# jayin92/Skyfall-GS

Measured on AMD Instinct MI355X. Metric: train-step Gaussians/s (fwd+bwd raster) @1080p, higher is better.
Workload: dtype f32; 1 GPU; configs[1]: synthetic cfg2 scene (SURVEY 8d), N=2000000 Gaussians/GPU, 1920x1080, z ~ U(250, 350), colors_precomp, kernel_size=0.1, subpixel_offset=zeros[H,W,2], dL/dimage and dL/ddepth ~ N(0,1)/P, seed=rank, one scene per GPU; N=2000000, width=1920, height=1080, N_vis=2000000, D_ref_16x16=5856939, D_binned_8x8=6945415, parallelism=scene-per-gpu x1, prewarm_steps=50, settle_steps=0, order=random

## Files before the change

### include/sfgs.h

```cpp
#ifndef SFGS_H
#define SFGS_H

#include <stddef.h>
#include <stdint.h>

#ifdef __cplusplus
extern "C" {
#endif

#define SFGS_ABI_VERSION 23

typedef enum SfgsStatus {
  SFGS_OK = 0,
  SFGS_E_ARG = -1,
  SFGS_E_HIP = -2,
  SFGS_E_CAPACITY = -3,
  SFGS_E_UNSUPPORTED = -4
} SfgsStatus;

#define SFGS_DEPTH_NORMALISED 0
#define SFGS_DEPTH_RAW 1

typedef struct SfgsFrame {
  uint32_t struct_size;
  int32_t image_height;
  int32_t image_width;
  float tanfovx;
  float tanfovy;
  float kernel_size;
  float scale_modifier;
  int32_t sh_degree;
  int32_t sh_coeffs;
  int32_t prefiltered;
// ... 54 lines not shown
  size_t geom_bytes;
  size_t tiles_bytes;
  size_t bins_bytes;
  size_t image_bytes;
  size_t dupgrad_bytes;
  int64_t coarse_bins;
} SfgsRasterSizes;

typedef struct SfgsRasterCounters {
  int64_t num_duplicates;
  int64_t num_duplicates_ref;
  int64_t num_visible;
  int64_t max_tile_list;
  int64_t overflow;
  int64_t max_coarse_bin;
  int64_t num_huge_splats;
  int64_t num_big_chunks;
  int64_t prev_valid;
  int64_t prev_long_tiles;
  int64_t prev_max_tile_list;
  int64_t prev_prefilled;
  int64_t prev_tiles_over_512;
  int64_t max_bin_items;
} SfgsRasterCounters;

int sfgs_abi_version(void);
const char* sfgs_last_error(void);

int sfgs_set_option(const char* key, const char* value);
const char* sfgs_get_option(const char* key);

int sfgs_profile_enable(int32_t on);
int sfgs_profile_select(uint64_t kernel_mask);
int sfgs_profile_kernel_count(void);
const char* sfgs_profile_kernel_name(int32_t id);
int sfgs_profile_collect(double* ms_sum, int64_t* launches, int32_t n);

int sfgs_box_probe(double* valu_tflops, double* sclk_mhz_effective, void* stream);

int sfgs_raster_sizes(int32_t N, int32_t W, int32_t H, int64_t D, int64_t coarse_capacity,
                      SfgsRasterSizes* out);
int64_t sfgs_raster_slot_capacity(int32_t W, int32_t H, int64_t num_duplicates);

int sfgs_raster_forward_plan(const SfgsFrame* frame, const SfgsGaussians* g, int32_t* radii,
                             void* geom, size_t geom_bytes, void* tiles, size_t tiles_bytes,
                             void* bins, size_t bins_bytes, int64_t dup_capacity,
// ... 243 lines not shown
```

### skyfall-gs_amd/csrc/api.cpp

```cpp
#include <hip/hip_runtime.h>
#include <stdarg.h>
#include <stdio.h>

#include <stdlib.h>
#include <string.h>

#include <atomic>
#include <mutex>
#include <vector>

#include "../../include/sfgs.h"
#include "sfgs_internal.h"

namespace sfgs {
static thread_local char g_err[512] = "";
void set_error(const char* fmt, ...) {
  va_list ap;
  va_start(ap, fmt);
  vsnprintf(g_err, sizeof(g_err), fmt, ap);
  va_end(ap);
}

struct OptSpec { const char* key; const char* env; const char* values[6]; };
static const OptSpec kOpts[OPT_COUNT] = {
    {"sort", "SFGS_SORT", {"auto", "fused", "fused1024", "split", "fused768", nullptr}},
    {"plan_scan", "SFGS_PLAN_SCAN", {"fused", "separate", nullptr}},
    {"binning", "SFGS_BINNING", {"auto", "direct", nullptr}},
    {"prefill", "SFGS_PREFILL", {"auto", "always", "never", nullptr}},
    {"knn", "SFGS_KNN", {"auto", "brute", nullptr}},
    {"tile_order", "SFGS_TILE_ORDER", {"auto", "always", "never", nullptr}}};
static std::atomic<int> g_opt[OPT_COUNT];
static int opt_value(int which, const char* v) {
  for (int i = 0; v && kOpts[which].values[i]; ++i)
    if (!strcmp(v, kOpts[which].values[i])) return i;
  return -1;
}
static const bool g_opt_init = [] {
  for (int k = 0; k < OPT_COUNT; ++k) {
    const int v = opt_value(k, getenv(kOpts[k].env));
    g_opt[k].store(v < 0 ? 0 : v, std::memory_order_relaxed);
  }
  return true;
}();
int option(int which) { return g_opt[which].load(std::memory_order_relaxed); }

static const char* const kKernelNames[KID_COUNT] = {
    "subpix_bound", "preprocess", "bin_count", "bin_rank", "bin_scatter", "plan_scan", "fine_bin", "sort_tiles_small", "sort_tiles_reg_long",
    "sort_tiles_lds", "composite_fwd", "composite_bwd", "preprocess_bwd", "ssim_fwd", "ssim_mean", "ssim_bwd",
    "knn_dist2", "prepass_fwd", "prepass_bwd", "filter3d", "densify_stats", "adam", "sh_eval_fwd", "sh_eval_bwd", "compact_scan", "compact_gather", "densify",
    "opacity_entropy_fwd", "opacity_entropy_final", "opacity_entropy_bwd",
    "loss_photo_fwd", "loss_depth_fwd", "loss_final", "loss_photo_bwd", "loss_depth_bwd"};

struct ProfRec { int id; hipEvent_t a, b; };
// ... 92 lines not shown
```

### skyfall-gs_amd/csrc/raster_fwd.hip

```cpp
#include <stdlib.h>
#include <string.h>

#include <algorithm>

#include <type_traits>

#include "act_math.h"
#include "sfgs_internal.h"

namespace sfgs {

constexpr int REG_SORT_SMALL = 512;
constexpr int REG_SORT_MAX = 1024;

__global__ void __launch_bounds__(256) subpix_bound_kernel(const float* __restrict__ subpix, int64_t n,
                                                           unsigned long long* __restrict__ hdr) {
  __shared__ float s_m[4];
  float m = 0.f;
  const int64_t n4 = (reinterpret_cast<uintptr_t>(subpix) & 15) ? 0 : (n >> 2);
  const float4* __restrict__ v4 = reinterpret_cast<const float4*>(subpix);
  for (int64_t i = (int64_t)blockIdx.x * blockDim.x + threadIdx.x; i < n4; i += (int64_t)gridDim.x * blockDim.x) {
    const float4 v = v4[i];
    m = fmaxf(fmaxf(m, fmaxf(fabsf(v.x), fabsf(v.y))), fmaxf(fabsf(v.z), fabsf(v.w)));
  }
// ... 894 lines not shown
}

template <int EPL, int SIZE, int STEP>
__device__ __forceinline__ void bitonic_steps(unsigned long long (&key)[EPL], unsigned (&pay)[EPL], int lane) {
  if constexpr (STEP == 0 || (SIZE >> (STEP + 1)) >= 1) {
    bitonic_stage<EPL, SIZE, STEP>(key, pay, lane);
    bitonic_steps<EPL, SIZE, STEP + 1>(key, pay, lane);
  }
}

template <int EPL, int SIZE>
__device__ __forceinline__ void bitonic_sizes(unsigned long long (&key)[EPL], unsigned (&pay)[EPL], int lane) {
  if constexpr (SIZE <= 64 * EPL) {
    bitonic_steps<EPL, SIZE, 0>(key, pay, lane);
    bitonic_sizes<EPL, SIZE * 2>(key, pay, lane);
  }
}

template <int EPL>
__device__ __forceinline__ void wave_bitonic_sort(unsigned long long (&key)[EPL], unsigned (&pay)[EPL], int lane) {
  bitonic_sizes<EPL, 2>(key, pay, lane);
}

template <int EPL>
__device__ __forceinline__ void store_list_entries(uint32_t* __restrict__ dst, const unsigned (&v)[EPL]) {
  if constexpr (EPL >= 4) {
#pragma unroll
    for (int i = 0; i < EPL / 4; ++i)
      reinterpret_cast<uint4*>(dst)[i] = make_uint4(v[4 * i], v[4 * i + 1], v[4 * i + 2], v[4 * i + 3]);
  } else if constexpr (EPL == 2) {
    *reinterpret_cast<uint2*>(dst) = make_uint2(v[0], v[1]);
  } else {
    dst[0] = v[0];
  }
}

template <int EPL>
__device__ __forceinline__ void sort_tile_in_registers(unsigned s, int L, int lane, const uint4* __restrict__ items,
                                                       uint32_t* __restrict__ sorted_id,
                                                       uint32_t* __restrict__ sorted_dup) {
  unsigned long long key[EPL];
  unsigned pay[EPL];
  uint4 it[EPL];
#pragma unroll
  for (int r = 0; r < EPL; ++r) it[r] = items[s + min(r * 64 + lane, L - 1)];
#pragma unroll
// ... 16 lines not shown
__global__ void __launch_bounds__(256)
sort_tiles_reg_kernel(int T8, const uint2* __restrict__ tile_range, const uint4* __restrict__ items,
                      uint32_t* __restrict__ sorted_id, uint32_t* __restrict__ sorted_dup,
                      const unsigned long long* __restrict__ hdr, unsigned long long* __restrict__ feedback) {
  if (feedback && blockIdx.x == 0 && threadIdx.x == 0) {
    feedback[FB_VALID] = 1ull;
    feedback[FB_LONG_TILES] = hdr[HDR_LONG_COUNT];
    feedback[FB_MAX_LIST] = hdr[HDR_MAX_LIST];
    feedback[FB_OVER_512] = hdr[HDR_LONG_COUNT];
  }
  const int t = blockIdx.x * 4 + (threadIdx.x >> 6), lane = threadIdx.x & 63;
  if (t >= T8) return;
  const uint2 tr = tile_range[t];
  const int L = (int)tr.y;
  if (L == 0 || L > REG_SORT_SMALL) return;
  if (L <= 64) sort_tile_in_registers<1>(tr.x, L, lane, items, sorted_id, sorted_dup);
  else if (L <= 128) sort_tile_in_registers<2>(tr.x, L, lane, items, sorted_id, sorted_dup);
  else if (L <= 256) sort_tile_in_registers<4>(tr.x, L, lane, items, sorted_id, sorted_dup);
  else sort_tile_in_registers<8>(tr.x, L, lane, items, sorted_id, sorted_dup);
}

template <int SS_CAP>
struct alignas(16) SelectSortLds {
  unsigned long long key[SS_CAP];
  uint32_t pay[SS_CAP];
  uint32_t pad_[4];
};


template <int SS_CAP>
__global__ void __launch_bounds__(256)
select_sort_kernel(int TX8, int TY8, int CX, int NCB, uint32_t* __restrict__ coarse_count,
                   const uint4* __restrict__ csr, const uint4* __restrict__ slabs, unsigned coarse_capacity,
                   unsigned long long slot_capacity,
                   uint2* __restrict__ tile_range, uint4* __restrict__ items, uint32_t* __restrict__ long_tiles,
                   unsigned long long* __restrict__ hdr, uint32_t* __restrict__ sorted_id,
                   uint32_t* __restrict__ sorted_dup) {
  __shared__ SelectSortLds<SS_CAP> lds_all[COARSE];
  __shared__ unsigned s_cnt[COARSE];
  const unsigned lb = xcd_chunked(blockIdx.x, (unsigned)NCB * COARSE, 8u * COARSE);
  const int cb = (int)(lb / COARSE), q = (int)(lb % COARSE);
  const int tid = threadIdx.x;
  const int wave = __builtin_amdgcn_readfirstlane(tid >> 6), lane = tid & 63;
  const int tx = (cb % CX) * COARSE + wave, ty = (cb / CX) * COARSE + q;
  if (ty >= TY8) return;
  const int t = ty * TX8 + tx;
  const int bit = q * COARSE + wave;
  uint32_t* line = coarse_count + (size_t)cb * CC_STRIDE;
  const BinItems slab = bin_items(line, csr, slabs, (size_t)cb, coarse_capacity);
  const unsigned n = slab.n;
  if (n == 0) { if (lane == 0 && tx < TX8) tile_range[t] = make_uint2(0u, 0u); return; }
  SelectSortLds<SS_CAP>& lds = lds_all[wave];
  if (tid < COARSE) s_cnt[tid] = 0u;
  __syncthreads();
  constexpr int R = 8;
  const unsigned rowmask = 0xfu << (q * COARSE);
  for (unsigned i0 = 0; i0 < n; i0 += 256u * R) {
    uint4 it[R];
#pragma unroll
    for (int k = 0; k < R; ++k) it[k] = slab[min(i0 + 256u * k + tid, n - 1u)];
#pragma unroll
    for (int k = 0; k < R; ++k) {
      unsigned m = i0 + 256u * k + tid < n ? it[k].w & rowmask : 0u;
      while (m) {
        const int b = __builtin_ctz(m);
        m &= m - 1;
        const unsigned pos = atomicAdd(&s_cnt[b - q * COARSE], 1u);
        if (pos < (unsigned)SS_CAP) {
          SelectSortLds<SS_CAP>& dst = lds_all[b - q * COARSE];
          dst.key[pos] = ((unsigned long long)it[k].y << 32) | it[k].x;
          dst.pay[pos] = it[k].z + (unsigned)__popc(it[k].w & ((1u << b) - 1u));
        }
      }
    }
  }
  __syncthreads();
  if (tx >= TX8) return;
  const unsigned below = (1u << bit) - 1u;
  const unsigned c = __builtin_amdgcn_readfirstlane((int)s_cnt[wave]);
  const unsigned long long bin_base = line[2];
  const unsigned need = bin_slots_needed(line[1]);
  const bool dropped = bin_base + need > slot_capacity;
  unsigned off = 0;
  if (lane == 0) {
    if (dropped) hdr[HDR_OVERFLOW] = 1ull;
    else if (c) {
      off = atomicAdd(&line[3], (c + LIST_ALIGN - 1) & ~(unsigned)(LIST_ALIGN - 1));
      atomicMax(&line[4], c);
      if (c > (unsigned)REG_SORT_SMALL) atomicAdd(&line[5], 1u);
    }
  }
  if (dropped || c == 0) { if (lane == 0) tile_range[t] = make_uint2(0u, 0u); return; }
  if (c <= (unsigned)SS_CAP) {
    const int L = (int)c;
    auto finish = [&](auto epl_tag) {
      constexpr int EPL = decltype(epl_tag)::value;
      unsigned long long key[EPL];
      unsigned pay[EPL];
#pragma unroll
      for (int r = 0; r < EPL; ++r) {
        const int i = r * 64 + lane;
        const unsigned long long k = lds.key[min(i, SS_CAP - 1)];
        const unsigned p = lds.pay[min(i, SS_CAP - 1)];
        key[r] = i < L ? k : ~0ull;
        pay[r] = i < L ? p : 0u;
      }
      wave_bitonic_sort<EPL>(key, pay, lane);
      const unsigned s = (unsigned)bin_base + (unsigned)__builtin_amdgcn_readfirstlane((int)off);
      if (lane == 0) tile_range[t] = make_uint2(s, c);
      if (lane * EPL < ((L + LIST_ALIGN - 1) & ~(LIST_ALIGN - 1))) {
        unsigned ids[EPL];
#pragma unroll
        for (int r = 0; r < EPL; ++r) ids[r] = (unsigned)(key[r] & 0xffffffffull);
        store_list_entries<EPL>(sorted_id + s + lane * EPL, ids);
        store_list_entries<EPL>(sorted_dup + s + lane * EPL, pay);
      }
    };
    if (L <= 64) finish(std::integral_constant<int, 1>{});
    else if (L <= 128) finish(std::integral_constant<int, 2>{});
    else if (L <= 256) finish(std::integral_constant<int, 4>{});
    else if (SS_CAP <= 512 || L <= 512) finish(std::integral_constant<int, 8>{});
    else if constexpr (SS_CAP > 512) finish(std::integral_constant<int, 16>{});
    return;
  }
  const unsigned s = (unsigned)bin_base + (unsigned)__builtin_amdgcn_readfirstlane((int)off);
  if (lane == 0) {
    tile_range[t] = make_uint2(s, c);
    long_tiles[atomicAdd(&hdr[HDR_LONG_COUNT], 1ull)] = (unsigned)t;
  }
  unsigned done = 0;
  for (unsigned i0 = 0; i0 < n; i0 += 64u * R) {
    uint4 lt[R];
#pragma unroll
    for (int k = 0; k < R; ++k) lt[k] = slab[min(i0 + 64u * k + lane, n - 1u)];
#pragma unroll
    for (int k = 0; k < R; ++k) {
      const bool hit = i0 + 64u * k + lane < n && ((lt[k].w >> bit) & 1u);
      const unsigned long long b = __ballot(hit);
      const unsigned pos = done + __builtin_amdgcn_mbcnt_hi((unsigned)(b >> 32), __builtin_amdgcn_mbcnt_lo((unsigned)b, 0u));
      if (hit) items[s + pos] = make_uint4(lt[k].x, lt[k].y, lt[k].z + (unsigned)__popc(lt[k].w & below), 0u);
      done += (unsigned)__popcll(b);
    }
  }
}

__device__ void list_stats(int NCB, uint32_t* __restrict__ coarse_count, unsigned long long* hdr,
                           unsigned long long* __restrict__ feedback) {
  __shared__ unsigned ls_part[4], ls_over[4];
  unsigned m = 0, over = 0;
  for (int i = threadIdx.x; i < NCB; i += 256) {
    m = max(m, coarse_count[(size_t)i * CC_STRIDE + 4]);
    over += coarse_count[(size_t)i * CC_STRIDE + 5];
  }
#pragma unroll
  for (int d = 32; d >= 1; d >>= 1) {
    m = max(m, (unsigned)__shfl_xor((int)m, d));
    over += (unsigned)__shfl_xor((int)over, d);
  }
  if ((threadIdx.x & 63) == 0) { ls_part[threadIdx.x >> 6] = m; ls_over[threadIdx.x >> 6] = over; }
  __syncthreads();
  if (threadIdx.x == 0) {
    const unsigned long long mx = max(max(ls_part[0], ls_part[1]), max(ls_part[2], ls_part[3]));
    hdr[HDR_MAX_LIST] = mx;
    if (feedback) {
      feedback[FB_VALID] = 1ull;
      feedback[FB_LONG_TILES] = hdr[HDR_LONG_COUNT];
      feedback[FB_MAX_LIST] = mx;
      feedback[FB_OVER_512] = (unsigned long long)ls_over[0] + ls_over[1] + ls_over[2] + ls_over[3];
    }
  }
  __syncthreads();
}

template <int EPL>
__global__ void __launch_bounds__(256)
sort_tiles_reg_long_kernel(const uint32_t* __restrict__ long_tiles, const unsigned long long* __restrict__ hdr,
                           const uint2* __restrict__ tile_range, const uint4* __restrict__ items,
                           uint32_t* __restrict__ sorted_id, uint32_t* __restrict__ sorted_dup) {
  const unsigned n_long = (unsigned)hdr[HDR_LONG_COUNT];
  const int wave = __builtin_amdgcn_readfirstlane((int)(threadIdx.x >> 6)), lane = threadIdx.x & 63;
  for (unsigned li = blockIdx.x * 4 + wave; li < n_long; li += gridDim.x * 4) {
    const uint2 tr = tile_range[long_tiles[li]];
    const int L = (int)tr.y;
    if (L > 32 * EPL && L <= 64 * EPL) sort_tile_in_registers<EPL>(tr.x, L, lane, items, sorted_id, sorted_dup);
  }
}
// ... 734 lines not shown
  const BinsView bv = bins_view(bins, dup_capacity, NCB, coarse_capacity);
  SFGS_CHECK_HIP(zero_head(tiles, tv.zero_bytes, stream));
  if (frame->subpixel_offset) {
    const int64_t n = (int64_t)W * H * 2;
    const int blocks = (int)std::max<int64_t>(1, std::min<int64_t>((n / 4 + 255) / 256, 512));
    hipLaunchKernelGGL(subpix_bound_kernel, dim3(blocks), dim3(256), 0, stream, frame->subpixel_offset, n, tv.hdr);
  }
  if (N > 0) hipLaunchKernelGGL(plan_merge_rec_kernel, dim3(2048), dim3(256), 0, stream, mp, gv.rec);
  hipLaunchKernelGGL(plan_merge_items_kernel, dim3((unsigned)NCB), dim3(256), 0, stream, mp, (unsigned)export_capacity,
                     (unsigned)coarse_capacity, tv.coarse_count, bv.slabs, tv.hdr);
  hipLaunchKernelGGL(bin_base_scan_kernel, dim3(1), dim3(1024), 0, stream, (int)NCB, tv.coarse_count, tv.hdr);
  SFGS_POST_LAUNCH("plan_merge", stream, frame->debug);
  return SFGS_OK;
}

static void unpack_counters(const unsigned long long* h, SfgsRasterCounters* out) {
  out->num_duplicates = (int64_t)h[HDR_D_EFF];
  out->num_duplicates_ref = (int64_t)h[HDR_D_REF];
  out->num_visible = (int64_t)h[HDR_N_VIS];
  out->max_tile_list = (int64_t)h[HDR_MAX_LIST];
  out->overflow = (int64_t)h[HDR_OVERFLOW];
  out->max_coarse_bin = (int64_t)h[HDR_MAX_COARSE];
  out->max_bin_items = (int64_t)h[HDR_MAX_BIN_ITEMS];
  out->num_huge_splats = (int64_t)h[HDR_BIG_COUNT];
  out->num_big_chunks = (int64_t)h[HDR_BIG_CHUNKS];
  out->prev_valid = out->prev_long_tiles = out->prev_max_tile_list = out->prev_prefilled = out->prev_tiles_over_512 = 0;
}

extern "C" int sfgs_raster_counters_decode(const void* host_128, SfgsRasterCounters* out) {
  SFGS_REQUIRE(host_128 && out, SFGS_E_ARG, "NULL argument");
  const unsigned long long* h = (const unsigned long long*)host_128;
  unsigned long long hdr[HDR_WORDS] = {0};
  for (int i = 0; i < 8; ++i) hdr[i] = h[i];
  hdr[HDR_BIG_COUNT] = h[8];
  hdr[HDR_BIG_CHUNKS] = h[9];
  unpack_counters(hdr, out);
  out->prev_valid = (int64_t)h[10];
  out->prev_long_tiles = (int64_t)h[11];
  out->prev_max_tile_list = (int64_t)h[12];
  out->prev_prefilled = (int64_t)h[13];
  out->prev_tiles_over_512 = (int64_t)h[14];
  out->max_bin_items = (int64_t)h[15];
  return SFGS_OK;
}

extern "C" int sfgs_raster_read_counters(const void* tiles, SfgsRasterCounters* out, void* stream_) {
// ... 25 lines not shown
                                          int64_t num_duplicates, float* out_color, float* out_depth, float* out_alpha,
                                          void* image, size_t image_sz, void* stream_) {
  if (int rc = check_frame(frame)) return rc;
  hipStream_t stream = (hipStream_t)stream_;
  const int W = frame->image_width, H = frame->image_height;
  const int64_t NCB = coarse_bins(W, H);
  SFGS_REQUIRE(N >= 0 && tiles && out_color && out_depth && out_alpha && bins, SFGS_E_ARG, "NULL argument");
  SFGS_REQUIRE(dup_capacity >= 0 && dup_capacity < (1ll << 32) && coarse_capacity >= 0, SFGS_E_ARG, "bad capacity");
  SFGS_REQUIRE(num_duplicates < 0 || sfgs_raster_slot_capacity(W, H, num_duplicates) <= dup_capacity, SFGS_E_CAPACITY,
               "%lld duplicates need %lld list slots, dup_capacity is %lld: redo the plan with larger blobs",
               (long long)num_duplicates, (long long)sfgs_raster_slot_capacity(W, H, num_duplicates),
               (long long)dup_capacity);
  SFGS_REQUIRE(bins_sz >= bins_bytes(dup_capacity, NCB, coarse_capacity), SFGS_E_CAPACITY,
               "bins blob: %zu bytes given, %zu needed", bins_sz, bins_bytes(dup_capacity, NCB, coarse_capacity));
  SFGS_REQUIRE(image == nullptr || image_sz >= image_bytes(W, H, dup_capacity), SFGS_E_CAPACITY, "image blob too small");
  const TilesView tv = tiles_view(tiles, W, H, N, nullptr);
  const GeomView gv = geom_view(const_cast<void*>(geom), N);
  const BinsView bv = bins_view_csr(bins, dup_capacity, NCB, coarse_capacity, N);
  const KFrame kf = make_kframe(frame);
  const int TX8 = tiles8_x(W), TY8 = tiles8_y(H), T8 = TX8 * TY8, CX = coarse_x(W);
  const int fused_cap = sort_fused(frame->launch_hints);
  const bool fused = fused_cap != 0;
  if (fused) {
    { ProfScope ps_(KID_SORT_SMALL, stream);
      if (fused_cap > 768)
        hipLaunchKernelGGL(select_sort_kernel<1024>, dim3((unsigned)NCB * COARSE), dim3(256), 0, stream, TX8, TY8, CX,
                           (int)NCB, tv.coarse_count, bv.csr, bv.slabs, (unsigned)coarse_capacity,
                           (unsigned long long)dup_capacity, tv.tile_range, bv.items, tv.long_tiles, tv.hdr, bv.sorted_id,
                           bv.sorted_dup);
      else if (fused_cap > 512)
        hipLaunchKernelGGL(select_sort_kernel<768>, dim3((unsigned)NCB * COARSE), dim3(256), 0, stream, TX8, TY8, CX,
                           (int)NCB, tv.coarse_count, bv.csr, bv.slabs, (unsigned)coarse_capacity,
                           (unsigned long long)dup_capacity, tv.tile_range, bv.items, tv.long_tiles, tv.hdr, bv.sorted_id,
                           bv.sorted_dup);
      else
        hipLaunchKernelGGL(select_sort_kernel<512>, dim3((unsigned)NCB * COARSE), dim3(256), 0, stream, TX8, TY8, CX,
                           (int)NCB, tv.coarse_count, bv.csr, bv.slabs, (unsigned)coarse_capacity,
                           (unsigned long long)dup_capacity, tv.tile_range, bv.items, tv.long_tiles, tv.hdr, bv.sorted_id,
                           bv.sorted_dup); }
    SFGS_POST_LAUNCH("select_sort", stream, frame->debug);
  } else {
    { ProfScope ps_(KID_FINE_BIN, stream);
      hipLaunchKernelGGL(fine_bin_kernel, dim3((unsigned)NCB), dim3(256), 0, stream, TX8, TY8, CX, (int)NCB,
                         tv.coarse_count, bv.csr, bv.slabs, (unsigned)coarse_capacity, (unsigned long long)dup_capacity,
                         tv.tile_range, bv.items, tv.long_tiles, tv.hdr); }
    SFGS_POST_LAUNCH("fine_bin", stream, frame->debug);
  }
  if (num_duplicates != 0) {
    if (!fused) {
      { ProfScope ps_(KID_SORT_SMALL, stream);
        hipLaunchKernelGGL(sort_tiles_reg_kernel, dim3((T8 + 3) / 4), dim3(256), 0, stream, T8, tv.tile_range, bv.items,
                           bv.sorted_id, bv.sorted_dup, (const unsigned long long*)tv.hdr,
                           (unsigned long long*)frame->feedback); }
      SFGS_POST_LAUNCH("sort_tiles_small", stream, frame->debug);
    }
    const int stats_bins = fused ? (int)NCB : 0;
    if (frame->launch_hints & SFGS_HINT_FEW_LONG_LISTS) {
      ProfScope ps_(KID_SORT_LDS, stream);
      hipLaunchKernelGGL(sort_tiles_long_kernel<SORT_CAP>, dim3(std::min(T8, 768)), dim3(256), 0, stream, REG_SORT_SMALL,
                         tv.long_tiles, tv.hdr, tv.tile_range, bv.items, bv.sorted_id, bv.sorted_dup, stats_bins,
                         tv.coarse_count, tv.hdr, (unsigned long long*)frame->feedback);
    } else {
// ... 88 lines not shown
```

### skyfall-gs_amd/csrc/raster_math.h

```cpp
#pragma once
#include <math.h>
#include <stdint.h>

#ifdef __HIPCC__
#define SFGS_HD __host__ __device__ __forceinline__
#else
#define SFGS_HD static inline
#endif

namespace sfgs {

constexpr int TILE_REF = 16;
constexpr int TILE_BIN = 8;
constexpr float LOG2E = 1.4426950408889634f;
constexpr float LN2 = 0.6931471805599453f;

struct FrameParams {
  int W, H;
  float tanfovx, tanfovy, kernel_size, scale_modifier;
  int sh_degree, sh_coeffs, depth_mode;
  float view[16], proj[16], campos[3], bg[3];
};

struct SplatRec {
// ... 3 lines not shown
  float depth, r;
  float g, b;
  float ex, ey;
};

struct Projected {
  bool visible;
  int radius;
  int rminx, rminy, rmaxx, rmaxy;
  float mx, my;
  float a, b, c;
  float a0, b0, c0;
  float cA, cB, cC;
  float coef;
  float tx, ty, tz;
  float cov3d[6];
};

SFGS_HD int f2i_sat(float v) {
  if (v >= 2147483520.0f) return 2147483647;
  if (v <= -2147483648.0f) return (-2147483647 - 1);
  return (int)v;
}
SFGS_HD int imin(int a, int b) { return a < b ? a : b; }
SFGS_HD int imax(int a, int b) { return a > b ? a : b; }

SFGS_HD void quat_to_rot(const float* q, float R[9]) {
  const float r = q[0], x = q[1], y = q[2], z = q[3];
  R[0] = 1.f - 2.f * (y * y + z * z);
  R[1] = 2.f * (x * y - r * z);
  R[2] = 2.f * (x * z + r * y);
  R[3] = 2.f * (x * y + r * z);
  R[4] = 1.f - 2.f * (x * x + z * z);
  R[5] = 2.f * (y * z - r * x);
  R[6] = 2.f * (x * z - r * y);
  R[7] = 2.f * (y * z + r * x);
  R[8] = 1.f - 2.f * (x * x + y * y);
}

SFGS_HD void cov3d_of(const float* s, float mod, const float* q, float cov[6]) {
  float R[9];
  quat_to_rot(q, R);
  const float S0 = mod * s[0], S1 = mod * s[1], S2 = mod * s[2];
  const float M0 = R[0] * S0, M1 = R[1] * S1, M2 = R[2] * S2;
  const float M3 = R[3] * S0, M4 = R[4] * S1, M5 = R[5] * S2;
  const float M6 = R[6] * S0, M7 = R[7] * S1, M8 = R[8] * S2;
// ... 625 lines not shown
```

### skyfall-gs_amd/csrc/sfgs_internal.h

```cpp
#pragma once
#include <hip/hip_runtime.h>
#include <stdint.h>
#include <stdio.h>

#include "../../include/sfgs.h"
#include "raster_math.h"

namespace sfgs {

void set_error(const char* fmt, ...);

#define SFGS_CHECK_HIP(expr)                                                              \
  do {                                                                                    \
    hipError_t e_ = (expr);                                                               \
    if (e_ != hipSuccess) {                                                               \
      sfgs::set_error("%s failed: %s (%s:%d)", #expr, hipGetErrorString(e_), __FILE__, __LINE__); \
      return SFGS_E_HIP;                                                                  \
    }                                                                                     \
  } while (0)

#define SFGS_REQUIRE(cond, code, ...)  \
  do {                                 \
    if (!(cond)) {                     \
      sfgs::set_error(__VA_ARGS__);    \
      return (code);                   \
    }                                  \
  } while (0)

enum KernelId {
  KID_SUBPIX = 0, KID_PREPROCESS, KID_BIN_COUNT, KID_BIN_RANK, KID_BIN_SCATTER, KID_PLAN_SCAN, KID_FINE_BIN, KID_SORT_SMALL, KID_SORT_REG_LONG, KID_SORT_LDS,
  KID_COMPOSITE_FWD, KID_COMPOSITE_BWD, KID_PREPROCESS_BWD, KID_SSIM_FWD, KID_SSIM_MEAN, KID_SSIM_BWD, KID_KNN, KID_PREPASS_FWD, KID_PREPASS_BWD, KID_FILTER3D, KID_DENSIFY_STATS, KID_ADAM, KID_SH_EVAL_FWD, KID_SH_EVAL_BWD, KID_COMPACT_SCAN, KID_COMPACT_GATHER, KID_DENSIFY,
  KID_OPACITY_ENTROPY_FWD, KID_OPACITY_ENTROPY_FINAL, KID_OPACITY_ENTROPY_BWD,
  KID_LOSS_PHOTO_FWD, KID_LOSS_DEPTH_FWD, KID_LOSS_FINAL, KID_LOSS_PHOTO_BWD, KID_LOSS_DEPTH_BWD,
  KID_COUNT
};
enum { OPT_SORT, OPT_PLAN_SCAN, OPT_BINNING, OPT_PREFILL, OPT_KNN, OPT_TILE_ORDER, OPT_COUNT };
enum { SORT_AUTO = 0, SORT_FUSED = 1, SORT_FUSED1024 = 2, SORT_SPLIT = 3, SORT_FUSED768 = 4 };
enum { PREFILL_AUTO = 0, PREFILL_ALWAYS = 1, PREFILL_NEVER = 2 };
int option(int which);
bool prof_enabled();
bool prof_selected(int id);
void* prof_begin(int id, hipStream_t stream);
void prof_end(void* token, hipStream_t stream);
struct ProfScope {
  void* tok; hipStream_t st;
  ProfScope(int id, hipStream_t s) : tok(prof_selected(id) ? prof_begin(id, s) : nullptr), st(s) {}
  ~ProfScope() { if (tok) prof_end(tok, st); }
};

#define SFGS_POST_LAUNCH(name, stream, debug)                                      \
  do {                                                                             \
    hipError_t e_ = hipGetLastError();                                             \
    if (e_ == hipSuccess && (debug)) e_ = hipStreamSynchronize(stream);            \
    if (e_ != hipSuccess) {                                                        \
      sfgs::set_error("kernel %s failed: %s", name, hipGetErrorString(e_));        \
      return SFGS_E_HIP;                                                           \
    }                                                                              \
  } while (0)

static inline size_t align_up(size_t v, size_t a) { return (v + a - 1) / a * a; }
// ... 36 lines not shown
  for (int i = 0; i < 3; ++i) { f.campos[i] = k.campos[i]; f.bg[i] = k.bg[i]; }
  return f;
}

constexpr int PRE_BLOCK = 256;
enum { FB_VALID = 0, FB_LONG_TILES = 1, FB_MAX_LIST = 2, FB_PREFILLED = 3, FB_OVER_512 = 4 };
constexpr int HDR_WORDS = 64;

enum HeaderSlot {
  HDR_D_EFF = 0,
  HDR_D_REF = 1,
  HDR_N_VIS = 2,
  HDR_MAX_LIST = 3,
  HDR_OVERFLOW = 4,
  HDR_SUBPIX_BOUND = 5,
  HDR_ITEM_ALLOC = 6,
  HDR_MAX_COARSE = 7,
  HDR_LONG_COUNT = 8,
  HDR_BIG_CHUNKS = 9,
  HDR_BIG_COUNT = 10,
  HDR_PREFILLED = 11,
  HDR_CSR_CURSOR = 12,
  HDR_MAX_BIN_ITEMS = 13,
  HDR_TILE_ORDER = 14
};

constexpr int REC_F4 = 3;

struct GeomView {
  float4* rec;
  uint2* dup;
  uint4* big_list;
  uint32_t* block_items;
};
constexpr int PAIRS_PER_BLOCK = PRE_BLOCK * 6;
static inline size_t pairs_bytes(int64_t N) {
  const int64_t NB = (N + PRE_BLOCK - 1) / PRE_BLOCK;
  return align_up((size_t)NB * PAIRS_PER_BLOCK * 16, 256);
}
static inline size_t geom_bytes(int64_t N) {
  const int64_t NB = (N + PRE_BLOCK - 1) / PRE_BLOCK;
  return align_up((size_t)N * 16 * REC_F4, 256) + align_up((size_t)N * 8, 256) + align_up((size_t)N * 16, 256) +
         align_up((size_t)NB * 4, 256);
}
static inline GeomView geom_view(void* base, int64_t N) {
  GeomView g;
  const int64_t NB = (N + PRE_BLOCK - 1) / PRE_BLOCK;
// ... 338 lines not shown
```

### skyfall-gs_amd/diff_gauss/__init__.py

```python
import os
from typing import NamedTuple, Optional

import torch
import torch.nn as nn

from sfgs import _lib as L
from sfgs import features as _features, max_radii as _max_radii, prepass, sh as _sh, viewdirs as _viewdirs
from sfgs import affinity as _affinity

__all__ = ["GaussianRasterizationSettings", "GaussianRasterizer", "rasterize_gaussians", "last_counters",
           "last_backward_hints", "collect_full_counters"]


class GaussianRasterizationSettings(NamedTuple):
    image_height: int
    image_width: int
    tanfovx: float
    tanfovy: float
    kernel_size: float
    subpixel_offset: Optional[torch.Tensor]
    bg: torch.Tensor
    scale_modifier: float
    viewmatrix: torch.Tensor
    projmatrix: torch.Tensor
# ... 271 lines not shown
                frame.feedback = hs["fb"].data_ptr()
            pin, ev, pin_ptr, ev_handle, cnt = _pinned_counters(dev, stream)
            outs_ptr = outs.data_ptr()
            plane = 4 * H * W
            tries, pool_grown, attempts = 0, False, 0
            while True:
                attempts += 1
                total = _layout(lib, N, W, H, cap, ccap, need_bwd)[0]
                if total > _scratch_budget(dev):
                    raise RuntimeError(f"rasterizer scratch of {total / 2**30:.1f} GiB exceeds half of the device memory "
                                       f"(duplicates {cap}, fullest coarse bin {ccap}, {ncb} bins)")
                scratch = torch.empty(total, dtype=torch.uint8, device=dev)
                frame.launch_hints = fwd_hints
                L.check(lib.sfgs_raster_forward(frame, gs, radii.data_ptr(), scratch.data_ptr(), total, cap, ccap,
                                                int(need_bwd), pin_ptr, ev_handle, outs_ptr, outs_ptr + 3 * plane,
                                                outs_ptr + 4 * plane, stream))
                ev.synchronize()
                L.check(lib.sfgs_raster_counters_decode(pin_ptr, cnt))
                if _stats["full"]:
                    full = L.SfgsRasterCounters()
                    tiles_off = _tiles_offset(lib, N, W, H, cap, ccap, need_bwd)
                    L.check(lib.sfgs_raster_read_counters(scratch.data_ptr() + tiles_off, L.C.byref(full), stream))
                    cnt.max_tile_list = full.max_tile_list
                D, cmax = int(cnt.num_duplicates), int(cnt.max_coarse_bin)
                if (fwd_hints & HINT_NO_HUGE_SPLATS) and cnt.num_huge_splats:
                    fwd_hints &= ~HINT_NO_HUGE_SPLATS
                    continue
                if not cnt.overflow and D + over <= cap and cmax <= ccap:
                    break
                tries += 1
                if tries > 24:
                    raise RuntimeError(f"rasterizer plan still overflows after {tries} attempts (duplicates {D}, capacity "
                                       f"{cap}, fullest coarse bin {cmax} of {ccap})")
                new_cap, new_ccap = max(cap, int(D * 1.25) + 1024 + over), max(ccap, int(cmax * 1.25) + 256)
                if (new_cap, new_ccap) == (cap, ccap):
                    new_cap = cap * 2
                    pool_grown = True
                cap, ccap = new_cap, new_ccap
            if hs is not None:
                if cnt.prev_valid:
                    hs["long"] = int(cnt.prev_long_tiles)
                    hs["maxlist"] = int(cnt.prev_max_tile_list)
                    hs["over512"] = int(cnt.prev_tiles_over_512)
                    if hs["prefill_ran"]:
                        hs["prefilled"] = _next_prefilled(hs["prefilled"], int(cnt.prev_prefilled) != 0)
                hs["huge"] = _next_huge(hs["huge"], int(cnt.num_huge_splats))
                hs["cmax"] = int(cnt.max_bin_items)
                hs["D"] = D
                hs["prefill_ran"] = False
            _cap_hint[(di, W, H)] = _next_capacities(cap, ccap, D, cmax, over, pool_grown)
            global _last_counters
            _last_counters = dict(num_duplicates=D, num_duplicates_ref=int(cnt.num_duplicates_ref),
                                  num_visible=int(cnt.num_visible), max_coarse_bin=cmax, max_bin_items=int(cnt.max_bin_items),
                                  num_huge_splats=int(cnt.num_huge_splats), num_big_chunks=int(cnt.num_big_chunks), plan_attempts=attempts,
                                  max_tile_list=int(cnt.max_tile_list), N=N, W=W, H=H, dup_capacity=cap,
                                  coarse_capacity=ccap, fwd_hints=int(fwd_hints))
        finally:
            if switch:
                torch.cuda.set_device(prev_dev)
        color, depth, alpha = outs.split_with_sizes((3, 1, 1))
        norm = _zero(dev).expand(3, H, W)
        ctx.mark_non_differentiable(radii, norm)
        ctx.set_materialize_grads(False)
        if need_bwd:
            ctx.st = (frame, gs, keep, cap, ccap, D, int(cnt.num_big_chunks), hkey, sh_coeffs, colors_precomp is not None,
                      shs is not None, opacities.dtype, total, settings, bool(sh_channel_major))
            ctx.save_for_backward(means3D, scales, rotations, opacities, colors_precomp, shs, radii, scratch, filter_3D,
                                  sh_dirs, shs_rest, sh_centers)
        return color, depth, norm, alpha, radii

    @staticmethod
    def backward(ctx, g_color, g_depth, g_norm, g_alpha, g_radii):
        lib = L.load()
        (means3D, scales, rotations, opacities, colors_precomp, shs, radii, scratch, filter_3D, sh_dirs,
         shs_rest, sh_centers) = ctx.saved_tensors
        (frame0, gs, keep, cap, ccap, ndup, big_chunks, hkey, K, has_colors, has_shs, opac_dtype, total, settings, sh_cm) = ctx.st
        dev = means3D.device
        di = dev.index
# ... 211 lines not shown
```

### skyfall-gs_amd/sfgs/_lib.py

```python
import ctypes as C
import os

_HERE = os.path.dirname(os.path.abspath(__file__))
LIB_PATH = os.environ.get("SFGS_LIB") or os.path.join(_HERE, "libsfgs.so")
ABI_VERSION = 23

SFGS_OK = 0
DEPTH_NORMALISED, DEPTH_RAW = 0, 1


class SfgsFrame(C.Structure):
    _fields_ = [("struct_size", C.c_uint32), ("image_height", C.c_int32), ("image_width", C.c_int32),
                ("tanfovx", C.c_float), ("tanfovy", C.c_float), ("kernel_size", C.c_float),
                ("scale_modifier", C.c_float), ("sh_degree", C.c_int32), ("sh_coeffs", C.c_int32),
                ("prefiltered", C.c_int32), ("debug", C.c_int32), ("depth_mode", C.c_int32),
                ("tile_row_begin", C.c_int32), ("tile_row_end", C.c_int32),
                ("subpixel_offset", C.c_void_p), ("bg", C.c_void_p), ("viewmatrix", C.c_void_p),
                ("projmatrix", C.c_void_p), ("campos", C.c_void_p), ("launch_hints", C.c_uint32),
                ("feedback", C.c_void_p)]


class SfgsGaussians(C.Structure):
    _fields_ = [("struct_size", C.c_uint32), ("count", C.c_int32), ("means3D", C.c_void_p), ("scales", C.c_void_p),
                ("rotations", C.c_void_p), ("opacities", C.c_void_p), ("colors_precomp", C.c_void_p),
                ("shs", C.c_void_p), ("filter_3D", C.c_void_p), ("raw_f64_mask", C.c_int32),
                ("sh_dirs", C.c_void_p), ("shs_channel_major", C.c_int32),
                ("shs_rest", C.c_void_p),
                ("sh_centers", C.c_void_p)]
# ... 68 lines not shown

class SfgsDsmViewArgs(C.Structure):
    _fields_ = [("struct_size", C.c_uint32), ("H", C.c_int32), ("W", C.c_int32), ("depth", C.c_void_p), ("mask", C.c_void_p),
                ("M", C.c_double * 9), ("c", C.c_double * 3), ("origin", C.c_double * 3), ("cx_pix", C.c_double),
                ("cy_pix", C.c_double), ("focal_x", C.c_double), ("focal_y", C.c_double), ("xoff", C.c_double),
                ("yoff_top", C.c_double), ("resolution", C.c_double), ("xsize", C.c_int32), ("ysize", C.c_int32),
                ("mode", C.c_int32), ("radius", C.c_int32)]


class SfgsDsmrArgs(C.Structure):
    _fields_ = [("struct_size", C.c_uint32), ("ref_h", C.c_int32), ("ref_w", C.c_int32), ("sec_h", C.c_int32),
                ("sec_w", C.c_int32), ("ref", C.c_void_p), ("sec", C.c_void_p), ("irange", C.c_int32), ("scaling", C.c_int32),
                ("init_dx", C.c_int32), ("init_dy", C.c_int32)]


DSM_MAX, DSM_MEAN = 0, 1


class SfgsRasterCounters(C.Structure):
    _fields_ = [("num_duplicates", C.c_int64), ("num_duplicates_ref", C.c_int64), ("num_visible", C.c_int64),
                ("max_tile_list", C.c_int64), ("overflow", C.c_int64), ("max_coarse_bin", C.c_int64),
                ("num_huge_splats", C.c_int64), ("num_big_chunks", C.c_int64), ("prev_valid", C.c_int64),
                ("prev_long_tiles", C.c_int64), ("prev_max_tile_list", C.c_int64), ("prev_prefilled", C.c_int64),
                ("prev_tiles_over_512", C.c_int64), ("max_bin_items", C.c_int64)]


_V, _I32, _I64, _SZ = C.c_void_p, C.c_int32, C.c_int64, C.c_size_t
SYMBOLS = {
    "sfgs_abi_version": (C.c_int, []),
    "sfgs_last_error": (C.c_char_p, []),
    "sfgs_profile_enable": (C.c_int, [_I32]),
    "sfgs_profile_select": (C.c_int, [C.c_uint64]),
    "sfgs_set_option": (C.c_int, [C.c_char_p, C.c_char_p]),
    "sfgs_get_option": (C.c_char_p, [C.c_char_p]),
    "sfgs_profile_kernel_count": (C.c_int, []),
    "sfgs_profile_kernel_name": (C.c_char_p, [_I32]),
    "sfgs_profile_collect": (C.c_int, [C.POINTER(C.c_double), C.POINTER(C.c_int64), _I32]),
    "sfgs_box_probe": (C.c_int, [C.POINTER(C.c_double), C.POINTER(C.c_double), _V]),
    "sfgs_raster_sizes": (C.c_int, [_I32, _I32, _I32, _I64, _I64, C.POINTER(SfgsRasterSizes)]),
    "sfgs_raster_slot_capacity": (C.c_int64, [_I32, _I32, _I64]),
    "sfgs_raster_forward_plan": (C.c_int, [C.POINTER(SfgsFrame), C.POINTER(SfgsGaussians), _V, _V, _SZ, _V, _SZ, _V, _SZ,
                                            _I64, _I64, _V, _V]),
    "sfgs_raster_counters_decode": (C.c_int, [_V, C.POINTER(SfgsRasterCounters)]),
    "sfgs_raster_read_counters": (C.c_int, [_V, C.POINTER(SfgsRasterCounters), _V]),
    "sfgs_raster_read_counters_pinned": (C.c_int, [_V, _V, C.POINTER(SfgsRasterCounters), _V]),
    "sfgs_raster_forward_render": (C.c_int, [C.POINTER(SfgsFrame), _I32, _V, _V, _V, _SZ, _I64, _I64, _I64, _V, _V, _V,
                                              _V, _SZ, _V]),
# ... 129 lines not shown
```

Baseline: 2.180 billion Gaussians/s.

## Sort per-tile lists with packed 32-bit depth-position keys in fused select sort

In the fused select-sort kernel, depth is rebased to the wave's minimum and packed with the list position into a single 32-bit key. Lists of up to 512 entries are then sorted with a 32-bit bitonic sort instead of a 64-bit key plus payload sort, which halves shuffle traffic and register use. The LDS layout is split into a depth array and an id/payload pair that is gathered after the sort. If the depth range does not fit or equal depths tie, the tile falls back to the wide sort, which is counted in a new header counter.

```diff
diff --git a/include/sfgs.h b/include/sfgs.h
--- a/include/sfgs.h
+++ b/include/sfgs.h
@@ -8,7 +8,7 @@
 extern "C" {
 #endif
 
-#define SFGS_ABI_VERSION 23
+#define SFGS_ABI_VERSION 24
 
 typedef enum SfgsStatus {
   SFGS_OK = 0,
@@ -109,6 +109,7 @@
   int64_t prev_prefilled;
   int64_t prev_tiles_over_512;
   int64_t max_bin_items;
+  int64_t sort_wide_tiles;
 } SfgsRasterCounters;
 
 int sfgs_abi_version(void);
diff --git a/skyfall-gs_amd/csrc/api.cpp b/skyfall-gs_amd/csrc/api.cpp
--- a/skyfall-gs_amd/csrc/api.cpp
+++ b/skyfall-gs_amd/csrc/api.cpp
@@ -28,7 +28,8 @@
     {"binning", "SFGS_BINNING", {"auto", "direct", nullptr}},
     {"prefill", "SFGS_PREFILL", {"auto", "always", "never", nullptr}},
     {"knn", "SFGS_KNN", {"auto", "brute", nullptr}},
-    {"tile_order", "SFGS_TILE_ORDER", {"auto", "always", "never", nullptr}}};
+    {"tile_order", "SFGS_TILE_ORDER", {"auto", "always", "never", nullptr}},
+    {"sort_key", "SFGS_SORT_KEY", {"auto", "wide", "narrow", nullptr}}};
 static std::atomic<int> g_opt[OPT_COUNT];
 static int opt_value(int which, const char* v) {
   for (int i = 0; v && kOpts[which].values[i]; ++i)
diff --git a/skyfall-gs_amd/csrc/raster_fwd.hip b/skyfall-gs_amd/csrc/raster_fwd.hip
--- a/skyfall-gs_amd/csrc/raster_fwd.hip
+++ b/skyfall-gs_amd/csrc/raster_fwd.hip
@@ -940,6 +940,64 @@
   bitonic_sizes<EPL, 2>(key, pay, lane);
 }
 
+template <int EPL, int SIZE, int STEP>
+__device__ __forceinline__ void bitonic_stage(unsigned (&key)[EPL], int lane) {
+  constexpr int mask = STEP == 0 ? SIZE - 1 : (SIZE >> (STEP + 1));
+  constexpr int rmask = mask & (EPL - 1);
+  constexpr int lmask = mask / EPL;
+  if constexpr (lmask == 0) {
+#pragma unroll
+    for (int r = 0; r < EPL; ++r) {
+      const int q = r ^ rmask;
+      if (q > r) {
+        const unsigned kr = key[r], kq = key[q];
+        key[r] = min(kr, kq); key[q] = max(kr, kq);
+      }
+    }
+  } else {
+    const bool upper = (lane & (lmask & ~(lmask >> 1))) != 0;
+    unsigned nk[EPL];
+#pragma unroll
+    for (int r = 0; r < EPL; ++r) {
+      const unsigned theirs = xor_shuffle<lmask>(key[r ^ rmask]);
+      nk[r] = upper ? max(key[r], theirs) : min(key[r], theirs);
+    }
+#pragma unroll
+    for (int r = 0; r < EPL; ++r) key[r] = nk[r];
+  }
+}
+
+template <int EPL, int SIZE, int STEP>
+__device__ __forceinline__ void bitonic_steps(unsigned (&key)[EPL], int lane) {
+  if constexpr (STEP == 0 || (SIZE >> (STEP + 1)) >= 1) {
+    bitonic_stage<EPL, SIZE, STEP>(key, lane);
+    bitonic_steps<EPL, SIZE, STEP + 1>(key, lane);
+  }
+}
+
+template <int EPL, int SIZE>
+__device__ __forceinline__ void bitonic_sizes(unsigned (&key)[EPL], int lane) {
+  if constexpr (SIZE <= 64 * EPL) {
+    bitonic_steps<EPL, SIZE, 0>(key, lane);
+    bitonic_sizes<EPL, SIZE * 2>(key, lane);
+  }
+}
+
+template <int EPL>
+__device__ __forceinline__ void wave_bitonic_sort(unsigned (&key)[EPL], int lane) {
+  bitonic_sizes<EPL, 2>(key, lane);
+}
+
+__device__ __forceinline__ unsigned wave_min_u32(unsigned v) {
+  v = min(v, xor_shuffle<1>(v));
+  v = min(v, xor_shuffle<2>(v));
+  v = min(v, xor_shuffle<7>(v));
+  v = min(v, xor_shuffle<15>(v));
+  const unsigned a = (unsigned)__builtin_amdgcn_readlane((int)v, 0), b = (unsigned)__builtin_amdgcn_readlane((int)v, 16);
+  const unsigned c = (unsigned)__builtin_amdgcn_readlane((int)v, 32), d = (unsigned)__builtin_amdgcn_readlane((int)v, 48);
+  return min(min(a, b), min(c, d));
+}
+
 template <int EPL>
 __device__ __forceinline__ void store_list_entries(uint32_t* __restrict__ dst, const unsigned (&v)[EPL]) {
   if constexpr (EPL >= 4) {
@@ -1002,8 +1060,8 @@
 
 template <int SS_CAP>
 struct alignas(16) SelectSortLds {
-  unsigned long long key[SS_CAP];
-  uint32_t pay[SS_CAP];
+  uint2 idp[SS_CAP];
+  uint32_t depth[SS_CAP];
   uint32_t pad_[4];
 };
 
@@ -1015,7 +1073,7 @@
                    unsigned long long slot_capacity,
                    uint2* __restrict__ tile_range, uint4* __restrict__ items, uint32_t* __restrict__ long_tiles,
                    unsigned long long* __restrict__ hdr, uint32_t* __restrict__ sorted_id,
-                   uint32_t* __restrict__ sorted_dup) {
+                   uint32_t* __restrict__ sorted_dup, int narrow) {
   __shared__ SelectSortLds<SS_CAP> lds_all[COARSE];
   __shared__ unsigned s_cnt[COARSE];
   const unsigned lb = xcd_chunked(blockIdx.x, (unsigned)NCB * COARSE, 8u * COARSE);
@@ -1048,8 +1106,8 @@
         const unsigned pos = atomicAdd(&s_cnt[b - q * COARSE], 1u);
         if (pos < (unsigned)SS_CAP) {
           SelectSortLds<SS_CAP>& dst = lds_all[b - q * COARSE];
-          dst.key[pos] = ((unsigned long long)it[k].y << 32) | it[k].x;
-          dst.pay[pos] = it[k].z + (unsigned)__popc(it[k].w & ((1u << b) - 1u));
+          dst.depth[pos] = it[k].y;
+          dst.idp[pos] = make_uint2(it[k].x, it[k].z + (unsigned)__popc(it[k].w & ((1u << b) - 1u)));
         }
       }
     }
@@ -1075,20 +1133,68 @@
     const int L = (int)c;
     auto finish = [&](auto epl_tag) {
       constexpr int EPL = decltype(epl_tag)::value;
+      const bool owns = lane * EPL < ((L + LIST_ALIGN - 1) & ~(LIST_ALIGN - 1));
+      if (narrow) {
+        constexpr int PB = SS_CAP <= 512 ? 9 : 10;
+        static_assert(64 * EPL <= (1 << PB), "a list position fits the key's low bits");
+        unsigned key[EPL];
+        unsigned lmin = 0xffffffffu;
+#pragma unroll
+        for (int r = 0; r < EPL; ++r) {
+          const int i = r * 64 + lane;
+          const unsigned d = lds.depth[min(i, SS_CAP - 1)];
+          key[r] = i < L ? d : 0xffffffffu;
+          lmin = min(lmin, key[r]);
+        }
+        const unsigned dmin = wave_min_u32(lmin);
+        bool bad = false;
+#pragma unroll
+        for (int r = 0; r < EPL; ++r) {
+          const int i = r * 64 + lane;
+          bad |= i < L && !sortkey_fits(dmin, key[r], PB);
+          key[r] = i < L ? sortkey_pack(key[r], dmin, (unsigned)i, PB) : SORTKEY_PAD;
+        }
+        if (__ballot(bad) == 0ull) {
+          wave_bitonic_sort<EPL>(key, lane);
+          const unsigned next0 = (unsigned)__shfl_down((int)key[0], 1);
+          bool tie = lane < 63 && !sortkey_is_padding(next0) && sortkey_same_depth(key[EPL - 1], next0, PB);
+#pragma unroll
+          for (int r = 0; r + 1 < EPL; ++r)
+            tie |= !sortkey_is_padding(key[r + 1]) && sortkey_same_depth(key[r], key[r + 1], PB);
+          if (__ballot(tie) == 0ull) {
+            const unsigned s = (unsigned)bin_base + (unsigned)__builtin_amdgcn_readfirstlane((int)off);
+            if (lane == 0) tile_range[t] = make_uint2(s, c);
+            if (owns) {
+              unsigned ids[EPL], pay[EPL];
+#pragma unroll
+              for (int r = 0; r < EPL; ++r) {
+                const bool pad = sortkey_is_padding(key[r]);
+                const uint2 e = lds.idp[min(sortkey_pos(key[r], PB), (unsigned)SS_CAP - 1u)];
+                ids[r] = pad ? 0xffffffffu : e.x;
+                pay[r] = pad ? 0u : e.y;
+              }
+              store_list_entries<EPL>(sorted_id + s + lane * EPL, ids);
+              store_list_entries<EPL>(sorted_dup + s + lane * EPL, pay);
+            }
+            return;
+          }
+        }
+      }
+      if (lane == 0) atomicAdd(&line[8], 1u);
       unsigned long long key[EPL];
       unsigned pay[EPL];
 #pragma unroll
       for (int r = 0; r < EPL; ++r) {
         const int i = r * 64 + lane;
-        const unsigned long long k = lds.key[min(i, SS_CAP - 1)];
-        const unsigned p = lds.pay[min(i, SS_CAP - 1)];
-        key[r] = i < L ? k : ~0ull;
-        pay[r] = i < L ? p : 0u;
+        const unsigned d = lds.depth[min(i, SS_CAP - 1)];
+        const uint2 e = lds.idp[min(i, SS_CAP - 1)];
+        key[r] = i < L ? (((unsigned long long)d << 32) | e.x) : ~0ull;
+        pay[r] = i < L ? e.y : 0u;
       }
       wave_bitonic_sort<EPL>(key, pay, lane);
       const unsigned s = (unsigned)bin_base + (unsigned)__builtin_amdgcn_readfirstlane((int)off);
       if (lane == 0) tile_range[t] = make_uint2(s, c);
-      if (lane * EPL < ((L + LIST_ALIGN - 1) & ~(LIST_ALIGN - 1))) {
+      if (owns) {
         unsigned ids[EPL];
 #pragma unroll
         for (int r = 0; r < EPL; ++r) ids[r] = (unsigned)(key[r] & 0xffffffffull);
@@ -1126,22 +1232,25 @@
 
 __device__ void list_stats(int NCB, uint32_t* __restrict__ coarse_count, unsigned long long* hdr,
                            unsigned long long* __restrict__ feedback) {
-  __shared__ unsigned ls_part[4], ls_over[4];
-  unsigned m = 0, over = 0;
+  __shared__ unsigned ls_part[4], ls_over[4], ls_wide[4];
+  unsigned m = 0, over = 0, wide = 0;
   for (int i = threadIdx.x; i < NCB; i += 256) {
     m = max(m, coarse_count[(size_t)i * CC_STRIDE + 4]);
     over += coarse_count[(size_t)i * CC_STRIDE + 5];
+    wide += coarse_count[(size_t)i * CC_STRIDE + 8];
   }
 #pragma unroll
   for (int d = 32; d >= 1; d >>= 1) {
     m = max(m, (unsigned)__shfl_xor((int)m, d));
     over += (unsigned)__shfl_xor((int)over, d);
-  }
-  if ((threadIdx.x & 63) == 0) { ls_part[threadIdx.x >> 6] = m; ls_over[threadIdx.x >> 6] = over; }
+    wide += (unsigned)__shfl_xor((int)wide, d);
+  }
+  if ((threadIdx.x & 63) == 0) { ls_part[threadIdx.x >> 6] = m; ls_over[threadIdx.x >> 6] = over; ls_wide[threadIdx.x >> 6] = wide; }
   __syncthreads();
   if (threadIdx.x == 0) {
     const unsigned long long mx = max(max(ls_part[0], ls_part[1]), max(ls_part[2], ls_part[3]));
     hdr[HDR_MAX_LIST] = mx;
+    hdr[HDR_SORT_WIDE] = (unsigned long long)ls_wide[0] + ls_wide[1] + ls_wide[2] + ls_wide[3];
     if (feedback) {
       feedback[FB_VALID] = 1ull;
       feedback[FB_LONG_TILES] = hdr[HDR_LONG_COUNT];
@@ -1922,6 +2031,7 @@
   out->overflow = (int64_t)h[HDR_OVERFLOW];
   out->max_coarse_bin = (int64_t)h[HDR_MAX_COARSE];
   out->max_bin_items = (int64_t)h[HDR_MAX_BIN_ITEMS];
+  out->sort_wide_tiles = (int64_t)h[HDR_SORT_WIDE];
   out->num_huge_splats = (int64_t)h[HDR_BIG_COUNT];
   out->num_big_chunks = (int64_t)h[HDR_BIG_CHUNKS];
   out->prev_valid = out->prev_long_tiles = out->prev_max_tile_list = out->prev_prefilled = out->prev_tiles_over_512 = 0;
@@ -1993,22 +2103,23 @@
   const int fused_cap = sort_fused(frame->launch_hints);
   const bool fused = fused_cap != 0;
   if (fused) {
+    const int narrow = option(OPT_SORT_KEY) == SORT_KEY_NARROW || (option(OPT_SORT_KEY) == SORT_KEY_AUTO && fused_cap <= 512);
     { ProfScope ps_(KID_SORT_SMALL, stream);
       if (fused_cap > 768)
         hipLaunchKernelGGL(select_sort_kernel<1024>, dim3((unsigned)NCB * COARSE), dim3(256), 0, stream, TX8, TY8, CX,
                            (int)NCB, tv.coarse_count, bv.csr, bv.slabs, (unsigned)coarse_capacity,
                            (unsigned long long)dup_capacity, tv.tile_range, bv.items, tv.long_tiles, tv.hdr, bv.sorted_id,
-                           bv.sorted_dup);
+                           bv.sorted_dup, narrow);
       else if (fused_cap > 512)
         hipLaunchKernelGGL(select_sort_kernel<768>, dim3((unsigned)NCB * COARSE), dim3(256), 0, stream, TX8, TY8, CX,
                            (int)NCB, tv.coarse_count, bv.csr, bv.slabs, (unsigned)coarse_capacity,
                            (unsigned long long)dup_capacity, tv.tile_range, bv.items, tv.long_tiles, tv.hdr, bv.sorted_id,
-                           bv.sorted_dup);
+                           bv.sorted_dup, narrow);
       else
         hipLaunchKernelGGL(select_sort_kernel<512>, dim3((unsigned)NCB * COARSE), dim3(256), 0, stream, TX8, TY8, CX,
                            (int)NCB, tv.coarse_count, bv.csr, bv.slabs, (unsigned)coarse_capacity,
                            (unsigned long long)dup_capacity, tv.tile_range, bv.items, tv.long_tiles, tv.hdr, bv.sorted_id,
-                           bv.sorted_dup); }
+                           bv.sorted_dup, narrow); }
     SFGS_POST_LAUNCH("select_sort", stream, frame->debug);
   } else {
     { ProfScope ps_(KID_FINE_BIN, stream);
diff --git a/skyfall-gs_amd/csrc/raster_math.h b/skyfall-gs_amd/csrc/raster_math.h
--- a/skyfall-gs_amd/csrc/raster_math.h
+++ b/skyfall-gs_amd/csrc/raster_math.h
@@ -49,6 +49,19 @@
   if (v <= -2147483648.0f) return (-2147483647 - 1);
   return (int)v;
 }
+constexpr uint32_t SORTKEY_PAD = 0xffffffffu;
+SFGS_HD uint32_t sortkey_max_range(int pos_bits) { return (0xffffffffu >> pos_bits) - 1u; }
+SFGS_HD bool sortkey_fits(uint32_t min_depth_bits, uint32_t max_depth_bits, int pos_bits) {
+  return max_depth_bits - min_depth_bits <= sortkey_max_range(pos_bits);
+}
+SFGS_HD uint32_t sortkey_pack(uint32_t depth_bits, uint32_t min_depth_bits, uint32_t pos, int pos_bits) {
+  return ((depth_bits - min_depth_bits) << pos_bits) | pos;
+}
+SFGS_HD uint32_t sortkey_pos(uint32_t key, int pos_bits) { return key & ((1u << pos_bits) - 1u); }
+SFGS_HD uint32_t sortkey_rel(uint32_t key, int pos_bits) { return key >> pos_bits; }
+SFGS_HD bool sortkey_is_padding(uint32_t key) { return key == SORTKEY_PAD; }
+SFGS_HD bool sortkey_same_depth(uint32_t a, uint32_t b, int pos_bits) { return ((a ^ b) >> pos_bits) == 0u; }
+
 SFGS_HD int imin(int a, int b) { return a < b ? a : b; }
 SFGS_HD int imax(int a, int b) { return a > b ? a : b; }
 
diff --git a/skyfall-gs_amd/csrc/sfgs_internal.h b/skyfall-gs_amd/csrc/sfgs_internal.h
--- a/skyfall-gs_amd/csrc/sfgs_internal.h
+++ b/skyfall-gs_amd/csrc/sfgs_internal.h
@@ -34,8 +34,9 @@
   KID_LOSS_PHOTO_FWD, KID_LOSS_DEPTH_FWD, KID_LOSS_FINAL, KID_LOSS_PHOTO_BWD, KID_LOSS_DEPTH_BWD,
   KID_COUNT
 };
-enum { OPT_SORT, OPT_PLAN_SCAN, OPT_BINNING, OPT_PREFILL, OPT_KNN, OPT_TILE_ORDER, OPT_COUNT };
+enum { OPT_SORT, OPT_PLAN_SCAN, OPT_BINNING, OPT_PREFILL, OPT_KNN, OPT_TILE_ORDER, OPT_SORT_KEY, OPT_COUNT };
 enum { SORT_AUTO = 0, SORT_FUSED = 1, SORT_FUSED1024 = 2, SORT_SPLIT = 3, SORT_FUSED768 = 4 };
+enum { SORT_KEY_AUTO = 0, SORT_KEY_WIDE = 1, SORT_KEY_NARROW = 2 };
 enum { PREFILL_AUTO = 0, PREFILL_ALWAYS = 1, PREFILL_NEVER = 2 };
 int option(int which);
 bool prof_enabled();
@@ -118,7 +119,8 @@
   HDR_PREFILLED = 11,
   HDR_CSR_CURSOR = 12,
   HDR_MAX_BIN_ITEMS = 13,
-  HDR_TILE_ORDER = 14
+  HDR_TILE_ORDER = 14,
+  HDR_SORT_WIDE = 15
 };
 
 constexpr int REC_F4 = 3;
diff --git a/skyfall-gs_amd/diff_gauss/__init__.py b/skyfall-gs_amd/diff_gauss/__init__.py
--- a/skyfall-gs_amd/diff_gauss/__init__.py
+++ b/skyfall-gs_amd/diff_gauss/__init__.py
@@ -317,6 +317,7 @@
                     tiles_off = _tiles_offset(lib, N, W, H, cap, ccap, need_bwd)
                     L.check(lib.sfgs_raster_read_counters(scratch.data_ptr() + tiles_off, L.C.byref(full), stream))
                     cnt.max_tile_list = full.max_tile_list
+                    cnt.sort_wide_tiles = full.sort_wide_tiles
                 D, cmax = int(cnt.num_duplicates), int(cnt.max_coarse_bin)
                 if (fwd_hints & HINT_NO_HUGE_SPLATS) and cnt.num_huge_splats:
                     fwd_hints &= ~HINT_NO_HUGE_SPLATS
@@ -348,7 +349,7 @@
             _last_counters = dict(num_duplicates=D, num_duplicates_ref=int(cnt.num_duplicates_ref),
                                   num_visible=int(cnt.num_visible), max_coarse_bin=cmax, max_bin_items=int(cnt.max_bin_items),
                                   num_huge_splats=int(cnt.num_huge_splats), num_big_chunks=int(cnt.num_big_chunks), plan_attempts=attempts,
-                                  max_tile_list=int(cnt.max_tile_list), N=N, W=W, H=H, dup_capacity=cap,
+                                  max_tile_list=int(cnt.max_tile_list), sort_wide_tiles=int(cnt.sort_wide_tiles), N=N, W=W, H=H, dup_capacity=cap,
                                   coarse_capacity=ccap, fwd_hints=int(fwd_hints))
         finally:
             if switch:
diff --git a/skyfall-gs_amd/sfgs/_lib.py b/skyfall-gs_amd/sfgs/_lib.py
--- a/skyfall-gs_amd/sfgs/_lib.py
+++ b/skyfall-gs_amd/sfgs/_lib.py
@@ -3,7 +3,7 @@
 
 _HERE = os.path.dirname(os.path.abspath(__file__))
 LIB_PATH = os.environ.get("SFGS_LIB") or os.path.join(_HERE, "libsfgs.so")
-ABI_VERSION = 23
+ABI_VERSION = 24
 
 SFGS_OK = 0
 DEPTH_NORMALISED, DEPTH_RAW = 0, 1
@@ -118,7 +118,7 @@
                 ("max_tile_list", C.c_int64), ("overflow", C.c_int64), ("max_coarse_bin", C.c_int64),
                 ("num_huge_splats", C.c_int64), ("num_big_chunks", C.c_int64), ("prev_valid", C.c_int64),
                 ("prev_long_tiles", C.c_int64), ("prev_max_tile_list", C.c_int64), ("prev_prefilled", C.c_int64),
-                ("prev_tiles_over_512", C.c_int64), ("max_bin_items", C.c_int64)]
+                ("prev_tiles_over_512", C.c_int64), ("max_bin_items", C.c_int64), ("sort_wide_tiles", C.c_int64)]
 
 
 _V, _I32, _I64, _SZ = C.c_void_p, C.c_int32, C.c_int64, C.c_size_t
```

Result: faster. 2.213 billion Gaussians/s (median of 6 runs) (+1.5%).
